# maxsonate/video-diffusion-nnx

Measured on AMD Instinct MI355X. Metric: denoised frames/sec, 16fx64x64 1000-step DDPM, higher is better.
Workload: dtype bf16; 1 GPU; config_v2_2 (north-star shape): Unet3D dim=64 C=1, 16f x 64x64, DDPM T=1000 p_sample_loop (UNet forward + p_sample per step, hipGraph replay); value = n_gpus*B*F/(T*s_per_step); batch_per_gpu=64, parallelism=dp1 (independent samples, no collective), mfma_operands=bf16, storage=weights fp32 master, activations bf16, fp32 accumulate, process_group=none (single process)

## Files before the change

video_diffusion_nnx_amd/csrc/sla.hip:

```cpp
#include "vdx_common.h"
#include "vdx_internal.h"
#include <stdlib.h>

namespace vdx {

constexpr int SLA_PART = 32 * 32 + 64;

template <int MODE>
__global__ __launch_bounds__(256) void sla_ctx_kernel(const SlaArgs P) {
    using M = Mma<MODE>;
    constexpr int KT = M::KT, KC = M::KC, RS = ROW_STRIDE;
    constexpr int APIECES = KT / 4;
    constexpr int NCHN = 64 / KC;
    constexpr int RSE = NCHN * 64 + 16;

    extern __shared__ __attribute__((aligned(16))) char smem[];
    float* m_run = reinterpret_cast<float*>(smem);
    float* s_run = m_run + 32;
    float* alpha = s_run + 32;
    float* pm = alpha + 32;
    char* xs = smem + 1024;
    char* ws = xs + 64 * RS;
    char* eT = ws + 64 * RS;
    char* vT = eT + 32 * RSE;
// ... 51 lines not shown
        const int r0 = chunk * R + sub * 64;
        if (r0 >= P.N) break;
        f32x4 acc[2][2];
#pragma unroll
        for (int i = 0; i < 2; ++i) { acc[i][0] = f32x4{0.f, 0.f, 0.f, 0.f}; acc[i][1] = f32x4{0.f, 0.f, 0.f, 0.f}; }
        for (int kt = 0; kt < nkt; ++kt) {
            __syncthreads();
            xput();
            if (!w_resident) stage_w(kt);
            __syncthreads();
            {
                int nk = kt + 1, nr0 = r0;
                if (nk == nkt) { nk = 0; nr0 = r0 + 64; }
                if (nr0 < P.N && nr0 < (chunk + 1) * R) xfetch(nr0, nk);
            }
#pragma unroll
            for (int ch = 0; ch < 2; ++ch) {
                uint4 bf[2], af[2];
#pragma unroll
                for (int tn = 0; tn < 2; ++tn) bf[tn] = *reinterpret_cast<const uint4*>(xs + ((wr * 2 + tn) * 16 + lp) * RS + ch * 64 + q * 16);
#pragma unroll
                for (int tm = 0; tm < 2; ++tm) af[tm] = *reinterpret_cast<const uint4*>(ws + ((wc * 2 + tm) * 16 + lp) * RS + ch * 64 + q * 16);
#pragma unroll
                for (int tm = 0; tm < 2; ++tm)
#pragma unroll
                    for (int tn = 0; tn < 2; ++tn) M::mma(acc[tm][tn], af[tm], bf[tn]);
            }
        }
        bool rv[2];
#pragma unroll
        for (int tn = 0; tn < 2; ++tn) rv[tn] = (r0 + (wr * 2 + tn) * 16 + lp) < P.N;
        if (wc == 0) {
#pragma unroll
            for (int tm = 0; tm < 2; ++tm)
#pragma unroll
                for (int r = 0; r < 4; ++r) {
                    float mx = fmaxf(rv[0] ? acc[tm][0][r] : -1e30f, rv[1] ? acc[tm][1][r] : -1e30f);
                    mx = max16(mx);
                    if (lp == 0) pm[wr * 32 + tm * 16 + 4 * q + r] = mx;
                }
        }
        __syncthreads();
        if (tid < 32) {
            const float mc = fmaxf(pm[tid], pm[32 + tid]);
            const float mo = m_run[tid];
            const float mn = fmaxf(mo, mc);
            alpha[tid] = __expf(mo - mn);
            m_run[tid] = mn;
        }
        __syncthreads();
        if (wc == 0) {
#pragma unroll
            for (int tm = 0; tm < 2; ++tm)
#pragma unroll
                for (int r = 0; r < 4; ++r) {
                    const int d = tm * 16 + 4 * q + r;
                    const float mn = m_run[d];
                    float ssum = 0.f;
#pragma unroll
                    for (int tn = 0; tn < 2; ++tn) {
                        const float e = rv[tn] ? __expf(acc[tm][tn][r] - mn) : 0.f;
                        M::store1(eT + d * RSE, (wr * 2 + tn) * 16 + lp, e);
                        ssum += e;
                    }
                    ssum = reduce16(ssum);
                    if (lp == 0) pm[wr * 32 + d] = ssum;
                }
        } else {
#pragma unroll
            for (int tm = 0; tm < 2; ++tm)
#pragma unroll
                for (int r = 0; r < 4; ++r) {
                    const int e = tm * 16 + 4 * q + r;
#pragma unroll
                    for (int tn = 0; tn < 2; ++tn)
                        M::store1(vT + e * RSE, (wr * 2 + tn) * 16 + lp, rv[tn] ? acc[tm][tn][r] : 0.f);
                }
        }
        __syncthreads();
        if (tid < 32) s_run[tid] = s_run[tid] * alpha[tid] + pm[tid] + pm[32 + tid];
#pragma unroll
        for (int r = 0; r < 4; ++r) cacc[r] *= alpha[dt * 16 + 4 * q + r];
#pragma unroll
        for (int ch = 0; ch < NCHN; ++ch) {
            const uint4 a = *reinterpret_cast<const uint4*>(eT + (dt * 16 + lp) * RSE + ch * 64 + q * 16);
            const uint4 bv = *reinterpret_cast<const uint4*>(vT + (et * 16 + lp) * RSE + ch * 64 + q * 16);
            M::mma(cacc, a, bv);
        }
    }
    __syncthreads();
    float* part = P.part + ((size_t)(n * P.nchunk + chunk) * P.heads + h) * SLA_PART;
#pragma unroll
    for (int r = 0; r < 4; ++r) part[(dt * 16 + 4 * q + r) * 32 + et * 16 + lp] = cacc[r];
    if (tid < 32) { part[1024 + tid] = m_run[tid]; part[1056 + tid] = s_run[tid]; }
}

template <int MODE>
__global__ __launch_bounds__(256) void sla_combine_kernel(const float* __restrict__ part, void* __restrict__ ctxT, int nchunk, int heads) {
    using M = Mma<MODE>;
    const int nh = blockIdx.x;
    const int n = nh / heads, h = nh % heads;
    __shared__ float Mx[32], Sx[32];
    const int tid = threadIdx.x;
    if (tid < 32) {
        float mx = -1e30f;
        for (int c = 0; c < nchunk; ++c) mx = fmaxf(mx, part[((size_t)(n * nchunk + c) * heads + h) * SLA_PART + 1024 + tid]);
        float s = 0.f;
        for (int c = 0; c < nchunk; ++c) {
            const float* p = part + ((size_t)(n * nchunk + c) * heads + h) * SLA_PART;
            s += p[1056 + tid] * __expf(p[1024 + tid] - mx);
        }
        Mx[tid] = mx; Sx[tid] = s;
    }
    __syncthreads();
    for (int i = tid; i < 1024; i += 256) {
        const int d = i >> 5, e = i & 31;
        float v = 0.f;
        for (int c = 0; c < nchunk; ++c) {
            const float* p = part + ((size_t)(n * nchunk + c) * heads + h) * SLA_PART;
            v += p[i] * __expf(p[1024 + d] - Mx[d]);
        }
        v /= Sx[d];
        char* row = reinterpret_cast<char*>(ctxT) + ((size_t)nh * 32 + e) * 32 * M::ES;
        M::store1(row, d, v);
    }
}

template <int MODE, int TMO>
__global__ __launch_bounds__(256) void sla_out_kernel(const SlaArgs P) {
    using M = Mma<MODE>;
    constexpr int KT = M::KT, KC = M::KC, RS = ROW_STRIDE;
    constexpr int APIECES = KT / 4;
    constexpr int NCHD = 32 / KC;
    constexpr int RSQ = (MODE == MODE_F32) ? 160 : 80;
    constexpr int HD = 256;
    constexpr int RSO = HD * M::ES + 16;
    constexpr int NCHO = HD / KC;

    extern __shared__ __attribute__((aligned(16))) char smem[];
    char* xs = smem;
    char* ws = xs + 64 * RS;
    char* qb = smem;
    char* os = qb + 4 * 64 * RSQ;

    const int tid = threadIdx.x, lane = tid & 63, w = tid >> 6;
    const int lp = lane & 15, q = lane >> 4;
    const int tiles = (P.N + 63) / 64;
    const int n = blockIdx.x / tiles, r0 = (blockIdx.x % tiles) * 64;
    const size_t xbase = (size_t)n * P.N * P.C;
    const int nkt = P.CPad / KT;
    const char* wq = reinterpret_cast<const char*>(P.wq);
    const char* wo = reinterpret_cast<const char*>(P.wo);

    f32x4 acc[4][4];
#pragma unroll
    for (int i = 0; i < 4; ++i)
#pragma unroll
        for (int j = 0; j < 4; ++j) acc[i][j] = f32x4{0.f, 0.f, 0.f, 0.f};
    for (int kt = 0; kt < nkt; ++kt) {
        __syncthreads();
        for (int i = tid; i < 64 * APIECES; i += 256) {
            const int row = i / APIECES, pc = i % APIECES;
            const int c = kt * KT + pc * 4;
            float4 v = make_float4(0.f, 0.f, 0.f, 0.f);
            if (r0 + row < P.N && c < P.C) v = load4_f32_or_bf16(P.x, xbase + (size_t)(r0 + row) * P.C + c, P.io_bf16);
            M::store4(xs + row * RS, pc * 4, v);
        }
        for (int i = tid; i < 256 * 8; i += 256) {
            const int row = i >> 3, pc = i & 7;
            *reinterpret_cast<uint4*>(ws + row * RS + pc * 16) =
                *reinterpret_cast<const uint4*>(wq + ((size_t)row * P.CPad + (size_t)kt * KT) * M::ES + pc * 16);
        }
        __syncthreads();
#pragma unroll
        for (int ch = 0; ch < 2; ++ch) {
            uint4 bf[4], af[4];
#pragma unroll
            for (int tn = 0; tn < 4; ++tn) bf[tn] = *reinterpret_cast<const uint4*>(xs + (tn * 16 + lp) * RS + ch * 64 + q * 16);
#pragma unroll
            for (int tm = 0; tm < 4; ++tm) af[tm] = *reinterpret_cast<const uint4*>(ws + ((w * 4 + tm) * 16 + lp) * RS + ch * 64 + q * 16);
#pragma unroll
            for (int tm = 0; tm < 4; ++tm)
#pragma unroll
                for (int tn = 0; tn < 4; ++tn) M::mma(acc[tm][tn], af[tm], bf[tn]);
        }
    }
    __syncthreads();
    char* myq = qb + w * 64 * RSQ;
#pragma unroll
    for (int hh = 0; hh < 2; ++hh) {
        const int h = 2 * w + hh;
#pragma unroll
        for (int tn = 0; tn < 4; ++tn) {
            float mx = -1e30f;
#pragma unroll
            for (int t2 = 0; t2 < 2; ++t2)
#pragma unroll
                for (int r = 0; r < 4; ++r) mx = fmaxf(mx, acc[2 * hh + t2][tn][r]);
            mx = max_q(mx);
            float e[2][4], sum = 0.f;
#pragma unroll
            for (int t2 = 0; t2 < 2; ++t2)
#pragma unroll
                for (int r = 0; r < 4; ++r) { e[t2][r] = __expf(acc[2 * hh + t2][tn][r] - mx); sum += e[t2][r]; }
            sum = reduce_q(sum);
            const float inv = 1.0f / sum;
#pragma unroll
            for (int t2 = 0; t2 < 2; ++t2)
                M::store4(myq + (tn * 16 + lp) * RSQ, t2 * 16 + 4 * q, make_float4(e[t2][0] * inv, e[t2][1] * inv, e[t2][2] * inv, e[t2][3] * inv));
        }
        __syncthreads();
        const char* ct = reinterpret_cast<const char*>(P.ctxT) + (size_t)(n * P.heads + h) * 32 * 32 * M::ES;
#pragma unroll
        for (int et = 0; et < 2; ++et) {
            f32x4 o[4];
#pragma unroll
            for (int tn = 0; tn < 4; ++tn) o[tn] = f32x4{0.f, 0.f, 0.f, 0.f};
#pragma unroll
            for (int ch = 0; ch < NCHD; ++ch) {
                const uint4 a = *reinterpret_cast<const uint4*>(ct + (size_t)(et * 16 + lp) * 32 * M::ES + ch * 64 + q * 16);
#pragma unroll
                for (int tn = 0; tn < 4; ++tn) {
                    const uint4 bq = *reinterpret_cast<const uint4*>(myq + (tn * 16 + lp) * RSQ + ch * 64 + q * 16);
                    M::mma(o[tn], a, bq);
                }
            }
#pragma unroll
            for (int tn = 0; tn < 4; ++tn)
                M::store4(os + (tn * 16 + lp) * RSO, h * 32 + et * 16 + 4 * q, make_float4(o[tn][0], o[tn][1], o[tn][2], o[tn][3]));
        }
        __syncthreads();
    }
    f32x4 oacc[TMO][4];
#pragma unroll
    for (int i = 0; i < TMO; ++i)
#pragma unroll
        for (int j = 0; j < 4; ++j) oacc[i][j] = f32x4{0.f, 0.f, 0.f, 0.f};
    for (int ch = 0; ch < NCHO; ++ch) {
        uint4 bf[4];
#pragma unroll
        for (int tn = 0; tn < 4; ++tn) bf[tn] = *reinterpret_cast<const uint4*>(os + (tn * 16 + lp) * RSO + ch * 64 + q * 16);
#pragma unroll
        for (int tmo = 0; tmo < TMO; ++tmo) {
            const int co = (w * TMO + tmo) * 16 + lp;
            uint4 a = make_uint4(0, 0, 0, 0);
            if (co < P.C) a = *reinterpret_cast<const uint4*>(wo + (size_t)co * HD * M::ES + ch * 64 + q * 16);
#pragma unroll
            for (int tn = 0; tn < 4; ++tn) M::mma(oacc[tmo][tn], a, bf[tn]);
        }
    }
#pragma unroll
    for (int tmo = 0; tmo < TMO; ++tmo) {
        const int co = (w * TMO + tmo) * 16 + 4 * q;
        if (co >= P.C) continue;
#pragma unroll
        for (int tn = 0; tn < 4; ++tn) {
            const int row = r0 + tn * 16 + lp;
            if (row >= P.N) continue;
            const float4 xr = load4_f32_or_bf16(P.x, xbase + (size_t)row * P.C + co, P.io_bf16);
            float4 v;
            v.x = oacc[tmo][tn][0] + xr.x; v.y = oacc[tmo][tn][1] + xr.y;
            v.z = oacc[tmo][tn][2] + xr.z; v.w = oacc[tmo][tn][3] + xr.w;
            store4_f32_or_bf16(P.y, xbase + (size_t)row * P.C + co, v, P.io_bf16);
        }
    }
}


template <int MODE, int NKT, bool IO16>
struct SlaTile {
    using M = Mma<MODE>;
    static_assert(!IO16 || MODE == MODE_BF16, "bf16 activation storage implies bf16 MFMA operands");
    static constexpr int PCH = IO16 ? 8 : 4;
    static constexpr int APIECES = M::KT / PCH;
    static constexpr int XP = 64 * APIECES * NKT / 512;
    static constexpr int PLANE = 64 * ROW_STRIDE;
    static constexpr int BUF = NKT * PLANE;
    float4 xpre[XP];
    __device__ __forceinline__ void fetch(const float* x, size_t xbase, int io_bf16, int r0, int N, int C, int tid) {
#pragma unroll
        for (int u = 0; u < XP; ++u) {
            const int i = tid + 512 * u;
            const int kt = i / (64 * APIECES), rem = i % (64 * APIECES);
            const int row = rem / APIECES, c = kt * M::KT + (rem % APIECES) * PCH;
            xpre[u] = make_float4(0.f, 0.f, 0.f, 0.f);
            if (r0 + row < N && c < C) {
                if (IO16) xpre[u] = *reinterpret_cast<const float4*>(reinterpret_cast<const char*>(x) + (xbase + (size_t)(r0 + row) * C + c) * 2);
                else xpre[u] = load4_f32_or_bf16(x, xbase + (size_t)(r0 + row) * C + c, io_bf16);
            }
        }
    }
    __device__ __forceinline__ void put(char* xs, int tid) const {
#pragma unroll
        for (int u = 0; u < XP; ++u) {
            const int i = tid + 512 * u;
            const int kt = i / (64 * APIECES), rem = i % (64 * APIECES);
            char* dst = xs + kt * PLANE + (rem / APIECES) * ROW_STRIDE;
            if (IO16) *reinterpret_cast<float4*>(dst + (rem % APIECES) * 16) = xpre[u];
            else M::store4(dst, (rem % APIECES) * 4, xpre[u]);
        }
    }
};

template <bool FULL>
__device__ __forceinline__ void ctx8_softmax_step(f32x4 (&acc)[2][4], float (&m_run)[2], float (&s_run)[2], f32x4 (&cacc)[2][2], int nleft) {
    constexpr float L2E = 1.44269504088896f;
#pragma unroll
    for (int dt = 0; dt < 2; ++dt) {
        if (!FULL) {
#pragma unroll
            for (int tn = 0; tn < 2; ++tn)
#pragma unroll
                for (int r = 0; r < 4; ++r) if (tn * 16 + r >= nleft) acc[tn][dt][r] = -1e30f;
        }
        float mx = fmaxf(fmaxf(fmaxf(acc[0][dt][0], acc[0][dt][1]), fmaxf(acc[0][dt][2], acc[0][dt][3])),
                         fmaxf(fmaxf(acc[1][dt][0], acc[1][dt][1]), fmaxf(acc[1][dt][2], acc[1][dt][3])));
        mx = max_q(mx);
        const float mn = fmaxf(m_run[dt], mx);
        const float alpha = __builtin_amdgcn_exp2f((m_run[dt] - mn) * L2E);
        m_run[dt] = mn;
        const float nb = -mn * L2E;
        float ssum = 0.f;
#pragma unroll
        for (int tn = 0; tn < 2; ++tn)
#pragma unroll
            for (int r = 0; r < 4; ++r) {
                float e = __builtin_amdgcn_exp2f(__builtin_fmaf(acc[tn][dt][r], L2E, nb));
                if (!FULL) e = (tn * 16 + r >= nleft) ? 0.f : e;
                acc[tn][dt][r] = e;
                ssum += e;
            }
        s_run[dt] = s_run[dt] * alpha + reduce_q(ssum);
#pragma unroll
        for (int et = 0; et < 2; ++et)
#pragma unroll
            for (int r = 0; r < 4; ++r) cacc[et][dt][r] *= alpha;
    }
}

template <int MODE, int NKT, bool IO16>
__global__ __launch_bounds__(512) void sla_ctx8_kernel(const SlaArgs P) {
    using M = Mma<MODE>;
    using T = SlaTile<MODE, NKT, IO16>;
    constexpr int RS = ROW_STRIDE;
    extern __shared__ __attribute__((aligned(16))) char smem[];
    const int tid = threadIdx.x, lane = tid & 63, h = tid >> 6;
    const int lp = lane & 15, q = lane >> 4;
    const int n = blockIdx.x / P.nchunk, chunk = blockIdx.x % P.nchunk;
    const int R = P.nsub * 64;
    const size_t xbase = (size_t)n * P.N * P.C;

    uint4 wf[NKT][2][4];
#pragma unroll
    for (int kt = 0; kt < NKT; ++kt)
#pragma unroll
        for (int ch = 0; ch < 2; ++ch)
#pragma unroll
            for (int tm = 0; tm < 4; ++tm) {
                const char* base = reinterpret_cast<const char*>(tm < 2 ? P.wk : P.wv);
                wf[kt][ch][tm] = *reinterpret_cast<const uint4*>(base + ((size_t)(h * 32 + (tm & 1) * 16 + lp) * P.CPad + kt * M::KT) * M::ES + ch * 64 + q * 16);
            }
    float m_run[2] = {-1e30f, -1e30f}, s_run[2] = {0.f, 0.f};
    f32x4 cacc[2][2];
#pragma unroll
    for (int i = 0; i < 2; ++i) { cacc[i][0] = f32x4{0.f, 0.f, 0.f, 0.f}; cacc[i][1] = f32x4{0.f, 0.f, 0.f, 0.f}; }

    T t;
    t.fetch(P.x, xbase, P.io_bf16, chunk * R, P.N, P.C, tid);
    t.put(smem, tid);
    __syncthreads();
    for (int sub = 0; sub < P.nsub; ++sub) {
        const int r0 = chunk * R + sub * 64;
        if (r0 >= P.N) break;
        const char* xs = smem + (sub & 1) * T::BUF;
        const bool more = (sub + 1 < P.nsub) && (r0 + 64 < P.N);
        if (more) t.fetch(P.x, xbase, P.io_bf16, r0 + 64, P.N, P.C, tid);
#pragma unroll
        for (int hf = 0; hf < 2; ++hf) {
            f32x4 acc[2][4];
#pragma unroll
            for (int i = 0; i < 2; ++i)
#pragma unroll
                for (int j = 0; j < 4; ++j) acc[i][j] = f32x4{0.f, 0.f, 0.f, 0.f};
#pragma unroll
            for (int kt = 0; kt < NKT; ++kt)
#pragma unroll
                for (int ch = 0; ch < 2; ++ch) {
                    uint4 xa[2];
#pragma unroll
                    for (int tn = 0; tn < 2; ++tn)
                        xa[tn] = *reinterpret_cast<const uint4*>(xs + kt * T::PLANE + ((hf * 2 + tn) * 16 + lp) * RS + ch * 64 + q * 16);
#pragma unroll
                    for (int tn = 0; tn < 2; ++tn)
#pragma unroll
                        for (int tm = 0; tm < 4; ++tm) M::mma(acc[tn][tm], xa[tn], wf[kt][ch][tm]);
                }
            if (r0 + 64 <= P.N) ctx8_softmax_step<true>(acc, m_run, s_run, cacc, 0);
            else ctx8_softmax_step<false>(acc, m_run, s_run, cacc, P.N - (r0 + hf * 32 + 4 * q));
#pragma unroll
            for (int tn = 0; tn < 2; ++tn)
#pragma unroll
                for (int et = 0; et < 2; ++et)
#pragma unroll
                    for (int dt = 0; dt < 2; ++dt) M::mma16(cacc[et][dt], acc[tn][2 + et], acc[tn][dt]);
        }
        if (more) t.put(smem + ((sub + 1) & 1) * T::BUF, tid);
        __syncthreads();
    }
    if (P.nchunk == 1) {
        char* ct = reinterpret_cast<char*>(P.ctxT) + (size_t)(n * P.heads + h) * 32 * 32 * M::ES;
#pragma unroll
        for (int dt = 0; dt < 2; ++dt) {
            const float inv = 1.0f / s_run[dt];
#pragma unroll
            for (int et = 0; et < 2; ++et)
#pragma unroll
                for (int r = 0; r < 4; ++r) M::store1(ct + (size_t)(et * 16 + 4 * q + r) * 32 * M::ES, dt * 16 + lp, cacc[et][dt][r] * inv);
        }
        return;
    }
    float* part = P.part + ((size_t)(n * P.nchunk + chunk) * P.heads + h) * SLA_PART;
#pragma unroll
    for (int et = 0; et < 2; ++et)
#pragma unroll
        for (int dt = 0; dt < 2; ++dt)
            *reinterpret_cast<float4*>(part + (dt * 16 + lp) * 32 + et * 16 + 4 * q) =
                make_float4(cacc[et][dt][0], cacc[et][dt][1], cacc[et][dt][2], cacc[et][dt][3]);
    if (q == 0) {
#pragma unroll
        for (int dt = 0; dt < 2; ++dt) { part[1024 + dt * 16 + lp] = m_run[dt]; part[1056 + dt * 16 + lp] = s_run[dt]; }
    }
}

template <int MODE, int NKT, int TMO, int TNO, bool IO16>
__global__ __launch_bounds__(512, NKT == 1 ? 4 : 2) void sla_out8_kernel(const SlaArgs P) {
    using M = Mma<MODE>;
    using T = SlaTile<MODE, NKT, IO16>;
    constexpr int RS = ROW_STRIDE, KC = M::KC, HD = 256;
    constexpr int RSO = HD * M::ES + 16;
    constexpr int NCHO = HD / KC;
    constexpr bool WO_RES = (TMO * NCHO <= 16);

    extern __shared__ __attribute__((aligned(16))) char smem[];
    char* os = smem + 2 * T::BUF;
    constexpr int RSY = NKT * M::KT * 4 + 16;
    char* ys = os + 64 * RSO;
    const int tid = threadIdx.x, lane = tid & 63, h = tid >> 6;
    const int lp = lane & 15, q = lane >> 4;
    const int n = blockIdx.x / P.nchunk, chunk = blockIdx.x % P.nchunk;
    const int R = P.nsub * 64;
    const size_t xbase = (size_t)n * P.N * P.C;

    uint4 wqf[NKT][2][2];
#pragma unroll
    for (int kt = 0; kt < NKT; ++kt)
#pragma unroll
        for (int ch = 0; ch < 2; ++ch)
#pragma unroll
            for (int tm = 0; tm < 2; ++tm)
                wqf[kt][ch][tm] = *reinterpret_cast<const uint4*>(reinterpret_cast<const char*>(P.wq) +
                    ((size_t)(h * 32 + tm * 16 + lp) * P.CPad + kt * M::KT) * M::ES + ch * 64 + q * 16);
    f32x4 cf[2][2];
    {
        const char* ct = reinterpret_cast<const char*>(P.ctxT) + (size_t)(n * P.heads + h) * 32 * 32 * M::ES;
#pragma unroll
        for (int et = 0; et < 2; ++et)
#pragma unroll
            for (int dt = 0; dt < 2; ++dt) cf[et][dt] = M::load_w4(ct + ((size_t)(et * 16 + lp) * 32 + dt * 16 + 4 * q) * M::ES);
    }
    const int cot0 = (TNO == 4) ? h * TMO : (TNO == 2) ? (h & 3) : (h & 1);
    const int tn0 = (TNO == 4) ? 0 : (TNO == 2) ? 2 * (h >> 2) : (h >> 1);
    const char* wo = reinterpret_cast<const char*>(P.wo);
    uint4 wof[WO_RES ? TMO : 1][WO_RES ? NCHO : 1];
    if (WO_RES) {
#pragma unroll
        for (int tmo = 0; tmo < TMO; ++tmo)
#pragma unroll
            for (int ch = 0; ch < NCHO; ++ch)
                wof[tmo][ch] = *reinterpret_cast<const uint4*>(wo + (size_t)((cot0 + tmo) * 16 + lp) * HD * M::ES + ch * 64 + q * 16);
    }

    T t;
    t.fetch(P.x, xbase, IO16 ? 1 : P.io_bf16, chunk * R, P.N, P.C, tid);
    t.put(smem, tid);
    __syncthreads();
    for (int sub = 0; sub < P.nsub; ++sub) {
        const int r0 = chunk * R + sub * 64;
        if (r0 >= P.N) break;
        const char* xs = smem + (sub & 1) * T::BUF;
        const bool more = (sub + 1 < P.nsub) && (r0 + 64 < P.N);
        float4 xcur[IO16 ? T::XP : 1];
        if (IO16) {
#pragma unroll
            for (int u = 0; u < T::XP; ++u) xcur[u] = t.xpre[u];
        }
        if (more) t.fetch(P.x, xbase, IO16 ? 1 : P.io_bf16, r0 + 64, P.N, P.C, tid);
        f32x4 acc[2][4];
#pragma unroll
        for (int i = 0; i < 2; ++i)
#pragma unroll
            for (int j = 0; j < 4; ++j) acc[i][j] = f32x4{0.f, 0.f, 0.f, 0.f};
#pragma unroll
        for (int kt = 0; kt < NKT; ++kt)
#pragma unroll
            for (int ch = 0; ch < 2; ++ch) {
                uint4 xb[4];
#pragma unroll
                for (int tn = 0; tn < 4; ++tn) xb[tn] = *reinterpret_cast<const uint4*>(xs + kt * T::PLANE + (tn * 16 + lp) * RS + ch * 64 + q * 16);
#pragma unroll
                for (int tm = 0; tm < 2; ++tm)
#pragma unroll
                    for (int tn = 0; tn < 4; ++tn) M::mma(acc[tm][tn], wqf[kt][ch][tm], xb[tn]);
            }
#pragma unroll
        for (int tn = 0; tn < 4; ++tn) {
            float mx = -1e30f;
#pragma unroll
            for (int tm = 0; tm < 2; ++tm)
#pragma unroll
                for (int r = 0; r < 4; ++r) mx = fmaxf(mx, acc[tm][tn][r]);
            mx = max_q(mx);
            const float nmx = -mx * 1.44269504088896f;
            float sum = 0.f;
#pragma unroll
            for (int tm = 0; tm < 2; ++tm)
#pragma unroll
                for (int r = 0; r < 4; ++r) { acc[tm][tn][r] = __builtin_amdgcn_exp2f(fmaf(acc[tm][tn][r], 1.44269504088896f, nmx)); sum += acc[tm][tn][r]; }
            const float inv = __builtin_amdgcn_rcpf(reduce_q(sum));
#pragma unroll
            for (int tm = 0; tm < 2; ++tm)
#pragma unroll
                for (int r = 0; r < 4; ++r) acc[tm][tn][r] *= inv;
        }
#pragma unroll
        for (int tn = 0; tn < 4; ++tn)
#pragma unroll
            for (int et = 0; et < 2; ++et) {
                f32x4 o = f32x4{0.f, 0.f, 0.f, 0.f};
#pragma unroll
                for (int dt = 0; dt < 2; ++dt) M::mma16(o, cf[et][dt], acc[dt][tn]);
                M::store4(os + (tn * 16 + lp) * RSO, h * 32 + et * 16 + 4 * q, make_float4(o[0], o[1], o[2], o[3]));
            }
        __syncthreads();
        f32x4 oacc[TMO][TNO];
#pragma unroll
        for (int i = 0; i < TMO; ++i)
#pragma unroll
            for (int j = 0; j < TNO; ++j) oacc[i][j] = f32x4{0.f, 0.f, 0.f, 0.f};
#pragma unroll
        for (int ch = 0; ch < NCHO; ++ch) {
            uint4 bf[TNO];
#pragma unroll
            for (int tn = 0; tn < TNO; ++tn) bf[tn] = *reinterpret_cast<const uint4*>(os + ((tn0 + tn) * 16 + lp) * RSO + ch * 64 + q * 16);
#pragma unroll
            for (int tmo = 0; tmo < TMO; ++tmo) {
                uint4 a;
                if (WO_RES) a = wof[tmo][ch];
                else a = *reinterpret_cast<const uint4*>(wo + (size_t)((cot0 + tmo) * 16 + lp) * HD * M::ES + ch * 64 + q * 16);
#pragma unroll
                for (int tn = 0; tn < TNO; ++tn) M::mma(oacc[tmo][tn], a, bf[tn]);
            }
        }
        if constexpr (IO16) {
#pragma unroll
            for (int tmo = 0; tmo < TMO; ++tmo)
#pragma unroll
                for (int tn = 0; tn < TNO; ++tn)
                    *reinterpret_cast<f32x4*>(ys + ((tn0 + tn) * 16 + lp) * RSY + ((cot0 + tmo) * 16 + 4 * q) * 4) = oacc[tmo][tn];
            if (more) t.put(smem + ((sub + 1) & 1) * T::BUF, tid);
            __syncthreads();
#pragma unroll
            for (int u = 0; u < T::XP; ++u) {
                const int i = tid + 512 * u;
                const int kt = i / (64 * T::APIECES), rem = i % (64 * T::APIECES);
                const int row = rem / T::APIECES, c = kt * M::KT + (rem % T::APIECES) * 8;
                if (r0 + row >= P.N || c >= P.C) continue;
                const float4 o4 = *reinterpret_cast<const float4*>(ys + row * RSY + c * 4), o5 = *reinterpret_cast<const float4*>(ys + row * RSY + c * 4 + 16);
                const unsigned x0 = __float_as_uint(xcur[u].x), x1 = __float_as_uint(xcur[u].y), x2 = __float_as_uint(xcur[u].z), x3 = __float_as_uint(xcur[u].w);
                uint4 w;
                w.x = pack_bf16x2(o4.x + __uint_as_float(x0 << 16), o4.y + __uint_as_float(x0 & 0xFFFF0000u));
                w.y = pack_bf16x2(o4.z + __uint_as_float(x1 << 16), o4.w + __uint_as_float(x1 & 0xFFFF0000u));
                w.z = pack_bf16x2(o5.x + __uint_as_float(x2 << 16), o5.y + __uint_as_float(x2 & 0xFFFF0000u));
                w.w = pack_bf16x2(o5.z + __uint_as_float(x3 << 16), o5.w + __uint_as_float(x3 & 0xFFFF0000u));
                *reinterpret_cast<uint4*>(reinterpret_cast<char*>(P.y) + (xbase + (size_t)(r0 + row) * P.C + c) * 2) = w;
            }
        } else {
#pragma unroll
            for (int tmo = 0; tmo < TMO; ++tmo) {
                const int co = (cot0 + tmo) * 16 + 4 * q;
#pragma unroll
                for (int tn = 0; tn < TNO; ++tn) {
                    const int row = r0 + (tn0 + tn) * 16 + lp;
                    if (row >= P.N) continue;
                    const float4 xr = load4_f32_or_bf16(P.x, xbase + (size_t)row * P.C + co, P.io_bf16);
                    store4_f32_or_bf16(P.y, xbase + (size_t)row * P.C + co,
                                       make_float4(oacc[tmo][tn][0] + xr.x, oacc[tmo][tn][1] + xr.y, oacc[tmo][tn][2] + xr.z, oacc[tmo][tn][3] + xr.w), P.io_bf16);
                }
            }
            if (more) t.put(smem + ((sub + 1) & 1) * T::BUF, tid);
            __syncthreads();
        }
    }
}

template <int DUMMY = 0>
__global__ __launch_bounds__(512) void sla_out_w_kernel(const SlaArgs P, const int frames_per_block) {
    using M = Mma<MODE_BF16>;
    constexpr int HD = 256, CRS = 72;
    extern __shared__ __attribute__((aligned(16))) char smem[];
    char* Wq = smem;
    char* Wo = Wq + HD * 128;
    char* Cx = Wo + 64 * 512;
    const int tid = threadIdx.x, lane = tid & 63;
    const int wave_u = __builtin_amdgcn_readfirstlane(tid >> 6);
    const int lp = lane & 15, q = lane >> 4;
    const int f0 = blockIdx.x * frames_per_block, f1 = min(f0 + frames_per_block, P.NF);
    if (f0 >= f1) return;

    for (int i = tid; i < HD * 8; i += 512) {
        const int r = i >> 3, c = i & 7;
        *reinterpret_cast<uint4*>(Wq + r * 128 + 16 * (c ^ (r & 7))) = *reinterpret_cast<const uint4*>(reinterpret_cast<const char*>(P.wq) + (size_t)r * 128 + c * 16);
    }
    for (int i = tid; i < 64 * 32; i += 512) {
        const int R = i >> 5, c = i & 31, hh = c >> 2, qq = c & 3;
        const int tile = R >> 4, ri = R & 15;
        const int co = 32 * (tile >> 1) + 8 * (ri >> 2) + 4 * (tile & 1) + (ri & 3);
        const char* src = reinterpret_cast<const char*>(P.wo) + (size_t)co * 512 + hh * 64 + qq * 8;
        const uint2 lo = *reinterpret_cast<const uint2*>(src), hi = *reinterpret_cast<const uint2*>(src + 32);
        *reinterpret_cast<uint4*>(Wo + R * 512 + 16 * (c ^ (R & 15))) = make_uint4(lo.x, lo.y, hi.x, hi.y);
    }
    auto load_ctx = [&](int f, int par) __attribute__((always_inline)) {
        const char* src = reinterpret_cast<const char*>(P.ctxT) + (size_t)f * (8 * 32 * 32 * 2);
        uint4 v[2];
#pragma unroll
        for (int u = 0; u < 2; ++u) v[u] = *reinterpret_cast<const uint4*>(src + (size_t)(tid + 512 * u) * 16);
#pragma unroll
        for (int u = 0; u < 2; ++u) {
            const int i = tid + 512 * u, row = i >> 2, pc = i & 3;
            char* d = Cx + par * (256 * CRS) + row * CRS + pc * 16;
            *reinterpret_cast<uint2*>(d) = make_uint2(v[u].x, v[u].y);
            *reinterpret_cast<uint2*>(d + 8) = make_uint2(v[u].z, v[u].w);
        }
    };
    load_ctx(f0, 0);
    __syncthreads();

    const int gpf = P.N >> 6;
    const char* const xg = reinterpret_cast<const char*>(P.x);
    char* const yg = reinterpret_cast<char*>(P.y);
    const unsigned loff = (unsigned)(lp * 64 + q * 8) * 2u;
    int wqo[2];
#pragma unroll
    for (int ch = 0; ch < 2; ++ch) wqo[ch] = lp * 128 + 16 * ((ch * 4 + q) ^ (lp & 7));
    const int woo = lp * 512;

    uint4 xn[4][2];
    auto fetch = [&](int f, int g) __attribute__((always_inline)) {
        const char* p = xg + ((size_t)f * P.N + (size_t)g * 64) * 128 + loff;
#pragma unroll
        for (int tn = 0; tn < 4; ++tn)
#pragma unroll
            for (int ch = 0; ch < 2; ++ch) xn[tn][ch] = *reinterpret_cast<const uint4*>(p + tn * (16 * 128) + ch * 64);
    };
    uint4 wcur[2][2], wnext[2][2];
    auto rd = [&](uint4 (&w)[2][2], const char* base) __attribute__((always_inline)) {
#pragma unroll
        for (int t = 0; t < 2; ++t)
#pragma unroll
            for (int ch = 0; ch < 2; ++ch) w[ch][t] = *reinterpret_cast<const uint4*>(base + t * 16 * 128 + wqo[ch]);
    };
    rd(wcur, Wq);
    if (wave_u < gpf) fetch(f0, wave_u);
    for (int f = f0; f < f1; ++f) {
        const int par = (f - f0) & 1;
        if (f + 1 < f1) load_ctx(f + 1, par ^ 1);
        const char* cimg = Cx + par * (256 * CRS);
        for (int g = wave_u; g < gpf; g += 8) {
            uint4 xc[4][2];
#pragma unroll
            for (int tn = 0; tn < 4; ++tn) { xc[tn][0] = xn[tn][0]; xc[tn][1] = xn[tn][1]; }
            if (g + 8 < gpf) fetch(f, g + 8);
            else if (f + 1 < f1 && wave_u < gpf) fetch(f + 1, wave_u);
            f32x4 yacc[4][4];
#pragma unroll
            for (int tn = 0; tn < 4; ++tn)
#pragma unroll
                for (int tile = 0; tile < 4; ++tile) yacc[tn][tile] = f32x4{0.f, 0.f, 0.f, 0.f};
#pragma unroll 1
            for (int h = 0; h < 8; ++h) {
                f32x4 acc[2][4];
#pragma unroll
                for (int i = 0; i < 2; ++i)
#pragma unroll
                    for (int j = 0; j < 4; ++j) acc[i][j] = f32x4{0.f, 0.f, 0.f, 0.f};
                {
                    const char* woh = Wo + woo + 16 * ((4 * h + q) ^ lp);
#pragma unroll
                    for (int tile = 0; tile < 4; ++tile) wnext[tile >> 1][tile & 1] = *reinterpret_cast<const uint4*>(woh + tile * 8192);
                }
                __builtin_amdgcn_sched_barrier(0);
#pragma unroll
                for (int ch = 0; ch < 2; ++ch)
#pragma unroll
                    for (int tm = 0; tm < 2; ++tm)
#pragma unroll
                        for (int tn = 0; tn < 4; ++tn) M::mma(acc[tm][tn], wcur[ch][tm], xc[tn][ch]);
                uint2 cf[2][2];
#pragma unroll
                for (int et = 0; et < 2; ++et)
#pragma unroll
                    for (int dt = 0; dt < 2; ++dt) cf[et][dt] = *reinterpret_cast<const uint2*>(cimg + (h * 32 + et * 16 + lp) * CRS + dt * 32 + q * 8);
// ... 384 lines not shown
```

Before: 49.63 frames/s.

## Restructure SLA ctx8 kernel with lazy softmax rescale and bf16 context MMA

Reworks the sparse-linear-attention context kernel so each 64-row subtile first computes V projections, packs them to bf16 and then computes K scores over all 64 rows at once. The online softmax only rescales when a wave's new max exceeds the running max by a threshold (ballot-gated), and the per-lane sum is reduced across quads once at the end instead of every step. The context accumulation uses bf16 16x16x16 MFMAs instead of fp32 mma16, and the tail subtile is peeled out of the main loop. Launch bounds now request higher occupancy, which trades per-thread register budget for the chance of spilling. Lazy rescale and bf16 packing change numerics slightly.

```diff
diff --git a/video_diffusion_nnx_amd/csrc/sla.hip b/video_diffusion_nnx_amd/csrc/sla.hip
--- a/video_diffusion_nnx_amd/csrc/sla.hip
+++ b/video_diffusion_nnx_amd/csrc/sla.hip
@@ -377,47 +377,129 @@
     }
 };
 
+constexpr float SLA_CTX8_THR = 8.0f;
+
+template <int MODE> struct Op16 {
+    using T = f32x4;
+    static __device__ __forceinline__ T pack(const f32x4& a) { return a; }
+    static __device__ __forceinline__ void pin(T&) {}
+    static __device__ __forceinline__ void mma(f32x4& acc, const T& a, const T& b) { Mma<MODE>::mma16(acc, a, b); }
+};
+template <> struct Op16<MODE_BF16> {
+    using T = uint2;
+    static __device__ __forceinline__ T pack(const f32x4& a) { return make_uint2(pack_bf16x2(a[0], a[1]), pack_bf16x2(a[2], a[3])); }
+    static __device__ __forceinline__ void pin(T& a) { asm volatile("" : "+v"(a.x), "+v"(a.y)); }
+    static __device__ __forceinline__ void mma(f32x4& acc, const T& a, const T& b) {
+        acc = __builtin_amdgcn_mfma_f32_16x16x16bf16_1k(__builtin_bit_cast(s16x4, a), __builtin_bit_cast(s16x4, b), acc, 0, 0, 0);
+    }
+};
+
+__device__ __forceinline__ float max16v(const f32x4& a, const f32x4& b, const f32x4& c, const f32x4& d) {
+    const float t0 = fmaxf(fmaxf(a[0], a[1]), a[2]), t1 = fmaxf(fmaxf(a[3], b[0]), b[1]), t2 = fmaxf(fmaxf(b[2], b[3]), c[0]);
+    const float t3 = fmaxf(fmaxf(c[1], c[2]), c[3]), t4 = fmaxf(fmaxf(d[0], d[1]), d[2]);
+    return fmaxf(fmaxf(fmaxf(t0, t1), t2), fmaxf(fmaxf(t3, t4), d[3]));
+}
+
 template <bool FULL>
-__device__ __forceinline__ void ctx8_softmax_step(f32x4 (&acc)[2][4], float (&m_run)[2], float (&s_run)[2], f32x4 (&cacc)[2][2], int nleft) {
+__device__ __forceinline__ void ctx8_softmax_step(f32x4 (&acc)[4][2], float (&m_run)[2], float (&s_run)[2], f32x4 (&cacc)[2][2], int nleft) {
     constexpr float L2E = 1.44269504088896f;
+    float mx[2];
 #pragma unroll
     for (int dt = 0; dt < 2; ++dt) {
         if (!FULL) {
 #pragma unroll
-            for (int tn = 0; tn < 2; ++tn)
+            for (int tn = 0; tn < 4; ++tn)
 #pragma unroll
                 for (int r = 0; r < 4; ++r) if (tn * 16 + r >= nleft) acc[tn][dt][r] = -1e30f;
         }
-        float mx = fmaxf(fmaxf(fmaxf(acc[0][dt][0], acc[0][dt][1]), fmaxf(acc[0][dt][2], acc[0][dt][3])),
-                         fmaxf(fmaxf(acc[1][dt][0], acc[1][dt][1]), fmaxf(acc[1][dt][2], acc[1][dt][3])));
-        mx = max_q(mx);
-        const float mn = fmaxf(m_run[dt], mx);
-        const float alpha = __builtin_amdgcn_exp2f((m_run[dt] - mn) * L2E);
-        m_run[dt] = mn;
-        const float nb = -mn * L2E;
-        float ssum = 0.f;
-#pragma unroll
-        for (int tn = 0; tn < 2; ++tn)
+        mx[dt] = max16v(acc[0][dt], acc[1][dt], acc[2][dt], acc[3][dt]);
+    }
+    const bool need = (mx[0] > m_run[0] + SLA_CTX8_THR) | (mx[1] > m_run[1] + SLA_CTX8_THR);
+    if (__builtin_amdgcn_ballot_w64(need) != 0) {
+#pragma unroll
+        for (int dt = 0; dt < 2; ++dt) {
+            const float mn = fmaxf(m_run[dt], max_q(mx[dt]));
+            const float alpha = __builtin_amdgcn_exp2f((m_run[dt] - mn) * L2E);
+            m_run[dt] = mn;
+            s_run[dt] *= alpha;
+#pragma unroll
+            for (int et = 0; et < 2; ++et) cacc[et][dt] *= alpha;
+        }
+    }
+#pragma unroll
+    for (int dt = 0; dt < 2; ++dt) {
+        const float nb = -m_run[dt] * L2E;
+        f32x4 sv = f32x4{0.f, 0.f, 0.f, 0.f};
+#pragma unroll
+        for (int tn = 0; tn < 4; ++tn) {
+            const f32x4 t = acc[tn][dt] * L2E + nb;
+            f32x4 e;
 #pragma unroll
             for (int r = 0; r < 4; ++r) {
-                float e = __builtin_amdgcn_exp2f(__builtin_fmaf(acc[tn][dt][r], L2E, nb));
-                if (!FULL) e = (tn * 16 + r >= nleft) ? 0.f : e;
-                acc[tn][dt][r] = e;
-                ssum += e;
-            }
-        s_run[dt] = s_run[dt] * alpha + reduce_q(ssum);
-#pragma unroll
-        for (int et = 0; et < 2; ++et)
-#pragma unroll
-            for (int r = 0; r < 4; ++r) cacc[et][dt][r] *= alpha;
-    }
+                e[r] = __builtin_amdgcn_exp2f(t[r]);
+                if (!FULL) e[r] = (tn * 16 + r >= nleft) ? 0.f : e[r];
+            }
+            acc[tn][dt] = e;
+            sv += e;
+        }
+        s_run[dt] += (sv[0] + sv[1]) + (sv[2] + sv[3]);
+    }
+}
+
+template <int MODE, int NKT, bool FULL>
+__device__ __forceinline__ void ctx8_subtile(const char* xs, const uint4 (&wf)[NKT][2][4], float (&m_run)[2], float (&s_run)[2], f32x4 (&cacc)[2][2],
+                                             int lp, int q, int nleft) {
+    using M = Mma<MODE>;
+    using O = Op16<MODE>;
+    constexpr int RS = ROW_STRIDE, PLANE = 64 * ROW_STRIDE;
+    typename O::T vop[4][2];
+    {
+        f32x4 av[4][2];
+#pragma unroll
+        for (int i = 0; i < 4; ++i) { av[i][0] = f32x4{0.f, 0.f, 0.f, 0.f}; av[i][1] = f32x4{0.f, 0.f, 0.f, 0.f}; }
+#pragma unroll
+        for (int kt = 0; kt < NKT; ++kt)
+#pragma unroll
+            for (int ch = 0; ch < 2; ++ch)
+#pragma unroll
+                for (int tn = 0; tn < 4; ++tn) {
+                    const uint4 xa = *reinterpret_cast<const uint4*>(xs + kt * PLANE + (tn * 16 + lp) * RS + ch * 64 + q * 16);
+#pragma unroll
+                    for (int et = 0; et < 2; ++et) M::mma(av[tn][et], xa, wf[kt][ch][2 + et]);
+                }
+#pragma unroll
+        for (int tn = 0; tn < 4; ++tn)
+#pragma unroll
+            for (int et = 0; et < 2; ++et) { vop[tn][et] = O::pack(av[tn][et]); O::pin(vop[tn][et]); }
+    }
+    f32x4 acc[4][2];
+#pragma unroll
+    for (int i = 0; i < 4; ++i) { acc[i][0] = f32x4{0.f, 0.f, 0.f, 0.f}; acc[i][1] = f32x4{0.f, 0.f, 0.f, 0.f}; }
+#pragma unroll
+    for (int kt = 0; kt < NKT; ++kt)
+#pragma unroll
+        for (int ch = 0; ch < 2; ++ch)
+#pragma unroll
+            for (int tn = 0; tn < 4; ++tn) {
+                const uint4 xa = *reinterpret_cast<const uint4*>(xs + kt * PLANE + (tn * 16 + lp) * RS + ch * 64 + q * 16);
+#pragma unroll
+                for (int dt = 0; dt < 2; ++dt) M::mma(acc[tn][dt], xa, wf[kt][ch][dt]);
+            }
+    ctx8_softmax_step<FULL>(acc, m_run, s_run, cacc, nleft);
+#pragma unroll
+    for (int tn = 0; tn < 4; ++tn)
+#pragma unroll
+        for (int dt = 0; dt < 2; ++dt) {
+            const typename O::T ek = O::pack(acc[tn][dt]);
+#pragma unroll
+            for (int et = 0; et < 2; ++et) O::mma(cacc[et][dt], vop[tn][et], ek);
+        }
 }
 
 template <int MODE, int NKT, bool IO16>
-__global__ __launch_bounds__(512) void sla_ctx8_kernel(const SlaArgs P) {
+__global__ __launch_bounds__(512, (NKT == 1 && IO16) ? 4 : 2) void sla_ctx8_kernel(const SlaArgs P) {
     using M = Mma<MODE>;
     using T = SlaTile<MODE, NKT, IO16>;
-    constexpr int RS = ROW_STRIDE;
     extern __shared__ __attribute__((aligned(16))) char smem[];
     const int tid = threadIdx.x, lane = tid & 63, h = tid >> 6;
     const int lp = lane & 15, q = lane >> 4;
@@ -444,44 +526,22 @@
     t.fetch(P.x, xbase, P.io_bf16, chunk * R, P.N, P.C, tid);
     t.put(smem, tid);
     __syncthreads();
-    for (int sub = 0; sub < P.nsub; ++sub) {
+    int sub = 0;
+    for (; sub < P.nsub; ++sub) {
         const int r0 = chunk * R + sub * 64;
-        if (r0 >= P.N) break;
-        const char* xs = smem + (sub & 1) * T::BUF;
+        if (r0 + 64 > P.N) break;
         const bool more = (sub + 1 < P.nsub) && (r0 + 64 < P.N);
         if (more) t.fetch(P.x, xbase, P.io_bf16, r0 + 64, P.N, P.C, tid);
-#pragma unroll
-        for (int hf = 0; hf < 2; ++hf) {
-            f32x4 acc[2][4];
-#pragma unroll
-            for (int i = 0; i < 2; ++i)
-#pragma unroll
-                for (int j = 0; j < 4; ++j) acc[i][j] = f32x4{0.f, 0.f, 0.f, 0.f};
-#pragma unroll
-            for (int kt = 0; kt < NKT; ++kt)
-#pragma unroll
-                for (int ch = 0; ch < 2; ++ch) {
-                    uint4 xa[2];
-#pragma unroll
-                    for (int tn = 0; tn < 2; ++tn)
-                        xa[tn] = *reinterpret_cast<const uint4*>(xs + kt * T::PLANE + ((hf * 2 + tn) * 16 + lp) * RS + ch * 64 + q * 16);
-#pragma unroll
-                    for (int tn = 0; tn < 2; ++tn)
-#pragma unroll
-                        for (int tm = 0; tm < 4; ++tm) M::mma(acc[tn][tm], xa[tn], wf[kt][ch][tm]);
-                }
-            if (r0 + 64 <= P.N) ctx8_softmax_step<true>(acc, m_run, s_run, cacc, 0);
-            else ctx8_softmax_step<false>(acc, m_run, s_run, cacc, P.N - (r0 + hf * 32 + 4 * q));
-#pragma unroll
-            for (int tn = 0; tn < 2; ++tn)
-#pragma unroll
-                for (int et = 0; et < 2; ++et)
-#pragma unroll
-                    for (int dt = 0; dt < 2; ++dt) M::mma16(cacc[et][dt], acc[tn][2 + et], acc[tn][dt]);
-        }
+        ctx8_subtile<MODE, NKT, true>(smem + (sub & 1) * T::BUF, wf, m_run, s_run, cacc, lp, q, 0);
         if (more) t.put(smem + ((sub + 1) & 1) * T::BUF, tid);
         __syncthreads();
     }
+    {
+        const int r0 = chunk * R + sub * 64;
+        if (sub < P.nsub && r0 < P.N) ctx8_subtile<MODE, NKT, false>(smem + (sub & 1) * T::BUF, wf, m_run, s_run, cacc, lp, q, P.N - (r0 + 4 * q));
+    }
+#pragma unroll
+    for (int dt = 0; dt < 2; ++dt) s_run[dt] = reduce_q(s_run[dt]);
     if (P.nchunk == 1) {
         char* ct = reinterpret_cast<char*>(P.ctxT) + (size_t)(n * P.heads + h) * 32 * 32 * M::ES;
 #pragma unroll
```

Result: no change. 50.02 frames/s, median of 6 (+0.8%).
